# refresh-bio/vclust

Measured on AMD Instinct MI355X. Metric: genome pairs/sec through prefilter+align (ani.tsv), higher is better.
Workload: dtype u64

## Files before the change

### include/vclust_gpu.h

```cpp
#ifndef VCLUST_GPU_H
#define VCLUST_GPU_H

#include <stdint.h>

#ifdef __cplusplus
extern "C" {
#endif

enum {
    VG_OK = 0, VG_EINVAL = -1, VG_EIO = -2, VG_ENODEV = -3, VG_EHIP = -4, VG_ENOMEM = -5,
    VG_EOVERFLOW = -6
};

const char* vg_version(void);
const char* vg_last_error(void);
void        vg_free(void* p);
int vg_device_count(void);
int vg_set_device(int device);
void vg_release_device_memory(void);
int vg_alloc_selftest(const int64_t* sizes, int n_sizes, int cycles);
int vg_copy(void* dst, const void* src, int64_t bytes, int to_host);

typedef struct vg_genomes vg_genomes;

// ... 18 lines not shown
typedef struct { uint32_t a, b, shared; } vg_pair_count;

int vg_kmer_shared(vg_genomes* g, int k, double fraction, int shard, int n_shards,
                   uint32_t min_shared, int64_t* set_sizes, vg_pair_count** pairs,
                   int64_t* n_pairs);
int vg_kmer_shared_new(vg_genomes* g, int n_db, int k, double fraction, uint32_t min_shared, int64_t* set_sizes,
                       vg_pair_count** pairs, int64_t* n_pairs);
void vg_set_new_path(int mode);
typedef struct {
    int accepted; int64_t P; int n_passes;
    int levels, total_bits, B1, B2;
    int st_tiles; int64_t n_st; int u_st, g_st;
    int tile32k, narrow, short_rec;
} vg_kmer_geometry_info;
int vg_kmer_geometry(const vg_genomes* g, int k, double fraction, int shard, int n_shards, vg_kmer_geometry_info* info);
int vg_kmer_geometry_at(int64_t padded_positions, int k, vg_kmer_geometry_info* info);
int vg_rowptr_inline_lo(int64_t entries, int64_t n_genomes, uint32_t* inline_lo);
int vg_kmer_set(vg_genomes* g, int idx, int k, double fraction, uint64_t** out, int64_t* n_out);

int vg_write_fltr(const vg_genomes* g, int k, double fraction, int min_kmers, double min_ident,
                  int max_seqs, const int64_t* set_sizes, const vg_pair_count* pairs,
                  int64_t n_pairs, const char* out_path);

int vg_filter_pairs(int k, int min_kmers, double min_ident, const int64_t* set_sizes, int64_t n_genomes,
                    const vg_pair_count* pairs, int64_t n_pairs, vg_pair_count** out, int64_t* n_out);

typedef struct {
    int    k;
    int    min_kmers;
    double min_ident;
// ... 291 lines not shown
```

### vclust_amd/_lib.py

```python
import collections
import ctypes as C
import os
import pathlib

PKG_DIR = pathlib.Path(__file__).resolve().parent
LIB_PATH = PKG_DIR / 'libvclust_gpu.so'


class VclustGpuError(RuntimeError):
    def __init__(self, code, msg):
        super().__init__(f'libvclust_gpu error {code}: {msg}')
        self.code = code


class PairCount(C.Structure):
    _fields_ = [('a', C.c_uint32), ('b', C.c_uint32), ('shared', C.c_uint32)]


class Task(C.Structure):
    _fields_ = [('q', C.c_uint32), ('r', C.c_uint32)]


class PairStat(C.Structure):
    _fields_ = [('n_match', C.c_uint32), ('aln_len', C.c_uint32), ('n_regions', C.c_uint32)]
# ... 179 lines not shown
    'vg_genomes_count': (C.c_int, [C.c_void_p]),
    'vg_genomes_total_len': (C.c_int64, [C.c_void_p]),
    'vg_genomes_lengths': (C.c_int, [C.c_void_p, P(C.c_int64)]),
    'vg_genomes_name': (C.c_char_p, [C.c_void_p, C.c_int]),
    'vg_genomes_codes': (C.c_int, [C.c_void_p, C.c_int, C.c_void_p]),
    'vg_genomes_to_device': (C.c_int, [C.c_void_p]),
    'vg_genomes_subset': (C.c_int, [C.c_void_p, P(C.c_int32), C.c_int, P(C.c_void_p)]),
    'vg_genomes_extend': (C.c_int, [C.c_void_p, C.c_void_p, P(C.c_int32), C.c_int]),
    'vg_genomes_truncate': (C.c_int, [C.c_void_p, C.c_int]),
    'vg_genomes_reserve': (C.c_int, [C.c_void_p, C.c_int64, C.c_int64]),
    'vg_kmer_shared': (C.c_int, [C.c_void_p, C.c_int, C.c_double, C.c_int, C.c_int, C.c_uint32,
                                 P(C.c_int64), P(P(PairCount)), P(C.c_int64)]),
    'vg_kmer_shared_new': (C.c_int, [C.c_void_p, C.c_int, C.c_int, C.c_double, C.c_uint32, P(C.c_int64), P(P(PairCount)), P(C.c_int64)]),
    'vg_kmer_geometry': (C.c_int, [C.c_void_p, C.c_int, C.c_double, C.c_int, C.c_int, P(KmerGeometry)]),
    'vg_kmer_geometry_at': (C.c_int, [C.c_int64, C.c_int, P(KmerGeometry)]),
    'vg_rowptr_inline_lo': (C.c_int, [C.c_int64, C.c_int64, P(C.c_uint32)]),
    'vg_kmer_set': (C.c_int, [C.c_void_p, C.c_int, C.c_int, C.c_double, P(P(C.c_uint64)), P(C.c_int64)]),
    'vg_filter_pairs': (C.c_int, [C.c_int, C.c_int, C.c_double, C.POINTER(C.c_int64), C.c_int64, C.POINTER(PairCount), C.c_int64,
                                  C.POINTER(C.POINTER(PairCount)), C.POINTER(C.c_int64)]),
    'vg_write_fltr': (C.c_int, [C.c_void_p, C.c_int, C.c_double, C.c_int, C.c_double, C.c_int,
                                P(C.c_int64), P(PairCount), C.c_int64, C.c_char_p]),
    'vg_prefilter': (C.c_int, [P(C.c_char_p), C.c_int, C.c_char_p, P(PrefilterParams)]),
    'vg_prefilter_new': (C.c_int, [P(C.c_char_p), C.c_int, P(C.c_char_p), C.c_int, C.c_char_p, P(PrefilterParams)]),
    'vg_set_process_ends_after_call': (None, [C.c_int]),
    'vg_set_lz_fit': (None, [P(LzFit)]),
    'vg_lz_align': (C.c_int, [C.c_void_p, P(Task), C.c_int64, P(LzParams), P(PairStat),
                              P(P(Region)), P(C.c_int64)]),
    'vg_align_order': (C.c_int, [C.c_void_p, P(C.c_int32)]),
    'vg_read_filter': (C.c_int, [C.c_void_p, C.c_char_p, C.c_double, P(P(PairCount)), P(C.c_int64)]),
    'vg_align_tasks': (C.c_int, [C.c_void_p, P(PairCount), C.c_int64, P(P(Task)), P(C.c_int64)]),
# ... 136 lines not shown
```

### vclust_amd/api.py

```python
import ctypes as C
import inspect

import numpy as np

from . import _lib
from ._lib import (ALIGN_FIELDS, ALIGN_OUTFMT, CLUSTER_ALGORITHMS, LINKAGE_ALGORITHMS, UPDATE_ALGORITHMS, ClusterStat, ClusterStats,
                   ClusterUpdateStats, DedupStats, DerepStats, DerepUpdateStats, KernelTime, LinkageStats, MclParams, MclStats, PairCount,
                   PairStat, Region, Task, as_dict, check, lz_params, path, path_array, ptr)
from .stages import (DEFAULT_LZ, align, align_params, cluster, cluster_stats, deduplicate as deduplicate_files, derep_params, dereplicate,
                     prefilter)


def _dtype(ctype):
    d = np.dtype(ctype)
    return np.dtype(d.descr) if d.names else d


PAIR_DTYPE, TASK_DTYPE, STAT_DTYPE, REGION_DTYPE, CLUSTER_STAT_DTYPE = (_dtype(t) for t in (PairCount, Task, PairStat, Region, ClusterStat))
LINKAGE_DTYPE = np.dtype([('node_a', '<i8'), ('node_b', '<i8'), ('similarity', '<f8'), ('size', '<i8'), ('object_a', '<i4'),
                          ('object_b', '<i4')])
AVERAGE_LINKAGE_DTYPE = np.dtype(LINKAGE_DTYPE.descr + [('sum', '<u8'), ('pairs', '<u8')])


def _input(x, ctype):
# ... 152 lines not shown
        pp, npairs = C.POINTER(PairCount)(), C.c_int64()
        sizes, = _filled(len(self), (C.c_int64,), lambda sp: check(self._lib.vg_kmer_shared(
            self._h, k, float(fraction), shard, n_shards, int(min_shared), sp, C.byref(pp), C.byref(npairs))))
        return sizes, _take(pp, npairs.value, PAIR_DTYPE)

    def kmer_shared_new(self, n_db, k=25, fraction=1.0, min_shared=1):
        pp, npairs = C.POINTER(PairCount)(), C.c_int64()
        sizes, = _filled(len(self), (C.c_int64,), lambda sp: check(self._lib.vg_kmer_shared_new(
            self._h, int(n_db), k, float(fraction), int(min_shared), sp, C.byref(pp), C.byref(npairs))))
        return sizes, _take(pp, npairs.value, PAIR_DTYPE)

    def kmer_geometry(self, k=25, fraction=1.0, shard=0, n_shards=1):
        info = _lib.KmerGeometry()
        check(self._lib.vg_kmer_geometry(self._h, int(k), float(fraction), int(shard), int(n_shards), C.byref(info)))
        return as_dict(info)

    def kmer_set(self, idx, k=25, fraction=1.0):
        p = C.POINTER(C.c_uint64)()
        n = C.c_int64()
        check(self._lib.vg_kmer_set(self._h, idx, k, float(fraction), C.byref(p), C.byref(n)))
        return _take(p, n.value, np.dtype('<u8'))

    def filter_pairs(self, set_sizes, pairs, k=25, min_kmers=20, min_ident=0.7):
        out, n = C.POINTER(PairCount)(), C.c_int64()
        check(self._lib.vg_filter_pairs(int(k), int(min_kmers), float(min_ident), *_input(set_sizes, C.c_int64), *_input(pairs, PairCount),
                                        C.byref(out), C.byref(n)))
        return _take(out, n.value, PAIR_DTYPE)

    def write_fltr(self, out_path, set_sizes, pairs, k=25, fraction=1.0, min_kmers=20, min_ident=0.7, max_seqs=0):
        check(self._lib.vg_write_fltr(self._h, k, float(fraction), int(min_kmers), float(min_ident), int(max_seqs),
# ... 273 lines not shown
```

### vclust_amd/csrc/vg_prefilter.hip

```cpp
#include "vg_common.h"
#include <functional>
#include <map>
#include <mutex>
#include <optional>
#include <rocprim/rocprim.hpp>
#include <algorithm>
#include <cmath>
#include <cstring>

namespace {

constexpr uint64_t SENT = ~0ULL;
constexpr uint32_t SCRAMBLE32 = 0x9E3779B1u;
__host__ __device__ __forceinline__ uint64_t scramble_key(uint64_t cano, int k) {
    const uint32_t L = (uint32_t)cano & ((1u << k) - 1u);
    const uint32_t H = (uint32_t)(cano >> k);
    return ((uint64_t)(H ^ ((L * SCRAMBLE32) >> (32 - k))) << k) | L;
}
__host__ __device__ __forceinline__ uint64_t unscramble_key(uint64_t key, int k) { return scramble_key(key, k); }
constexpr uint32_t DUP_BIT = 0x80000000u;
__device__ __forceinline__ uint32_t rowptr_inline(uint32_t partner) { return 0xFFFFFFFFu - partner; }
__device__ __forceinline__ uint32_t rowptr_partner_of_rs(uint32_t rs) { return 0xFFFFFFFEu - rs; }

__device__ __forceinline__ uint64_t mix64(uint64_t x) {
// ... 1263 lines not shown
                        const uint64_t r = short_rec_pack(key, short_kr, v[2] - grp_row0);
                        __builtin_memcpy(o_rec + 2 * dst, &r, 8);
                    } else __builtin_memcpy(o_rec + 3 * dst, v, 12);
                }
                lds_sync();
                cursors_advance(cursor, thist, nbins);
                lds_sync();
            }
        }
    }
}

constexpr int NT_TILE = 16384;
constexpr int NT_PER = NT_TILE / PT_THREADS;
constexpr int NT_MAXBINS = 2048;
template <bool SHORT>
__global__ void __launch_bounds__(PT_THREADS)
k_part_scatter2_narrow(const uint32_t* __restrict__ rec, int B1, int B2, int64_t n_units, const uint32_t* __restrict__ Ts, lvl2_tab L,
                       uint32_t* __restrict__ o_rec, int narrow_shift) {
    __shared__ uint2 s_rec[NT_TILE];
    __shared__ uint32_t thist[NT_MAXBINS], tstart[NT_MAXBINS], cursor[NT_MAXBINS];
    __shared__ uint32_t s_wave[16];
    const int nbins = 1 << B2;
    const int lane = threadIdx.x & 63, wv = threadIdx.x >> 6;
    for (int64_t u = blockIdx.x; u < n_units; u += gridDim.x) {
        uint32_t b1, U; int64_t s0, s1;
        lvl2_unit(L, u, &b1, &U, &s0, &s1);
        uint32_t gbase = 0, gb[3] = {0, 0, 0};
        uint32_t grow0 = 0, grow1 = 0, grow2 = 0, grow3 = 0;
        if (SHORT) {
            lvl2_groups(L, b1, U, s1, &gbase, gb);
            if (L.wbase) {
                const int64_t w0 = (int64_t)(gbase >> 6), gw = SR_GROUP_WORDS;
                grow0 = L.wbase[min(w0, L.W)]; grow1 = L.wbase[min(w0 + gw, L.W)]; grow2 = L.wbase[min(w0 + 2 * gw, L.W)]; grow3 = L.wbase[min(w0 + 3 * gw, L.W)];
            }
        }
        lds_sync();
        for (int b = threadIdx.x; b < nbins; b += PT_THREADS) cursor[b] = Ts[((uint64_t)b1 * L.n_u + U) * nbins + b];
        for (int64_t t0 = s0; t0 < s1; t0 += NT_TILE) {
            for (int b = threadIdx.x; b < nbins; b += PT_THREADS) thist[b] = 0;
            lds_sync();
            uint32_t key[NT_PER], pay[NT_PER], br[NT_PER];
            if (SHORT) {
                uint4 rr[NT_PER / 2];
#pragma unroll
                for (int p = 0; p < NT_PER / 2; ++p) {
                    const int64_t i = t0 + 2 * ((int64_t)p * PT_THREADS + threadIdx.x);
                    rr[p] = make_uint4(0u, 0u, 0u, 0u);
                    if (i + 1 < s1) __builtin_memcpy(&rr[p], rec + 2 * i, 16);
                    else if (i < s1) __builtin_memcpy(&rr[p].x, rec + 2 * i, 8);
                }
#pragma unroll
                for (int p = 0; p < NT_PER / 2; ++p) {
// ... 33 lines not shown
                uint32_t cn[BPT], tot = 0;
#pragma unroll
                for (int v = 0; v < BPT; ++v) { const int b = BPT * (int)threadIdx.x + v; cn[v] = b < nbins ? thist[b] : 0u; tot += cn[v]; }
                uint32_t run = block_scan_1024(tot, s_wave, nullptr);
#pragma unroll
                for (int v = 0; v < BPT; ++v) { const int b = BPT * (int)threadIdx.x + v; if (b < nbins) tstart[b] = run; run += cn[v]; }
            }
            lds_sync();
#pragma unroll
            for (int j = 0; j < NT_PER; ++j) if (br[j] != 0xffffffffu) s_rec[tstart[br[j] & 0x7ffu] + (br[j] >> 11)] = make_uint2(key[j], pay[j]);
            lds_sync();
            const int per_wave = (nbins + 15) >> 4;
            for (int bb = wv * per_wave; bb < min(nbins, (wv + 1) * per_wave); bb += 8) {
                const int b = bb + (lane >> 3);
                const bool live = b < min(nbins, (wv + 1) * per_wave);
                const uint32_t st = live ? tstart[b] : 0u, cnt = live ? thist[b] : 0u;
                const uint64_t cur = live ? cursor[b] : 0ull;
                for (uint32_t i = (uint32_t)(lane & 7); __any(i < cnt); i += 8) {
                    if (i < cnt) { const uint2 v = s_rec[st + i]; __builtin_memcpy(o_rec + 2 * (cur + i), &v, 8); }
                }
            }
            lds_sync();
            for (int b = threadIdx.x; b < nbins; b += PT_THREADS) cursor[b] += thist[b];
            lds_sync();
        }
    }
}

constexpr int SC_SLAB = 128;
__global__ void __launch_bounds__(PT_THREADS)
k_scan_columns_a(const uint32_t* __restrict__ T, int64_t n_rows, int n_cols, uint32_t* __restrict__ S) {
    const int64_t r0 = (int64_t)blockIdx.x * SC_SLAB, r1 = min(n_rows, r0 + SC_SLAB);
    for (int c = threadIdx.x; c < n_cols; c += PT_THREADS) {
        uint32_t sum = 0;
        for (int64_t r = r0; r < r1; ++r) sum += T[r * n_cols + c];
        S[(int64_t)blockIdx.x * n_cols + c] = sum;
    }
}
__global__ void __launch_bounds__(PT_THREADS)
// ... 52 lines not shown
        uint32_t acc = run;
        for (int u = 0; u < n_u; ++u) { const uint32_t t = tab[(size_t)u * nb2 + c]; tab[(size_t)u * nb2 + c] = acc; acc += t; }
        run += tot[v];
    }
    if (b1 == nb1 - 1 && threadIdx.x == 0) boff[(size_t)nb1 * nb2] = off1[nb1];
}

constexpr int BK_PER = BK_CAP / BK_THREADS;
constexpr int BK_MAXBIN = 768;
template <bool NARROW, int THREADS, int SUBBITS>
__global__ void __launch_bounds__(THREADS)
k_bucket_runs(const uint32_t* __restrict__ rec, int stride ,
              const uint32_t* __restrict__ boff, int64_t n_buckets, int pbits, const uint32_t* __restrict__ blk2g, int blk_shift,
              uint32_t* __restrict__ gen, uint32_t* __restrict__ rowinfo, compact_map M, int* __restrict__ dup_per_genome,
              const uint32_t* __restrict__ bucket_list ,
              uint32_t* __restrict__ over_list, unsigned int* __restrict__ n_over, uint32_t inline_lo) {
    constexpr int BK_SUB = 1 << SUBBITS, CAP = THREADS * BK_PER;
    const uint32_t inline_rank = inline_lo ? 1u : 0u;
    static_assert(CAP <= 8192 && BK_MAXBIN <= 1024, "slot | rank << 13 of the run members");
    __shared__ uint32_t s_big;
    __shared__ uint64_t sk[CAP];
    __shared__ uint32_t sp[NARROW ? 1 : CAP];
    __shared__ uint32_t sgen[CAP];
    __shared__ uint32_t cnt[BK_SUB + 1], start[BK_SUB + 1];
    __shared__ uint32_t s_wave[THREADS / 64];
    const int lane = threadIdx.x & 63, wv = threadIdx.x >> 6;
    for (int64_t it = blockIdx.x; it < n_buckets; it += gridDim.x) {
        const int64_t bk = bucket_list ? (int64_t)bucket_list[it] : it;
        const uint32_t b0 = boff[bk], b1 = boff[bk + 1];
        const uint32_t n_u = b1 - b0;
        if (n_u <= 1) continue;
        if (n_u > (uint32_t)CAP) { if (threadIdx.x == 0) over_list[atomicAdd(n_over, 1u)] = (uint32_t)bk; continue; }
        const int n = (int)n_u;
        lds_sync();
        for (int b = threadIdx.x; b <= BK_SUB; b += THREADS) cnt[b] = 0;
        if (threadIdx.x == 0) s_big = 0;
        lds_sync();
        uint64_t key[BK_PER]; uint32_t pj[BK_PER]; uint32_t sb[BK_PER], ar[BK_PER];
        if (NARROW) {
            static_assert(BK_PER % 2 == 0, "pairs of records per thread");
#pragma unroll
            for (int p = 0; p < BK_PER / 2; ++p) {
                const int j = 2 * (p * THREADS + (int)threadIdx.x);
                uint4 rr = make_uint4(0u, 0u, 0u, 0u);
                if (j + 1 < n) __builtin_memcpy(&rr, rec + 2 * (uint64_t)(b0 + j), 16);
                else if (j < n) __builtin_memcpy(&rr.x, rec + 2 * (uint64_t)(b0 + j), 8);
#pragma unroll
                for (int h = 0; h < 2; ++h) {
                    const int q = 2 * p + h;
                    const uint32_t a = h ? rr.z : rr.x, pay = h ? rr.w : rr.y;
                    sb[q] = 0; ar[q] = 0; key[q] = 0; pj[q] = 0;
                    if (j + h < n) { pj[q] = pay; key[q] = ((uint64_t)a << 32) | pay; sb[q] = a >> (32 - SUBBITS); }
                }
            }
        } else {
#pragma unroll
            for (int q = 0; q < BK_PER; ++q) {
                const int j = q * THREADS + threadIdx.x;
                sb[q] = 0; ar[q] = 0; key[q] = 0; pj[q] = 0;
                if (j < n) {
                    const uint32_t* r = rec + (uint64_t)(b0 + j) * stride;
                    const uint32_t a = r[0], c = stride == 3 ? r[1] : 0u;
                    pj[q] = r[stride - 1];
                    key[q] = ((uint64_t)a << 32) | c;
                    sb[q] = (uint32_t)((key[q] << pbits) >> (64 - SUBBITS));
                }
            }
        }
        auto rec_of = [&](int q) -> int { return NARROW ? 2 * ((q >> 1) * THREADS + (int)threadIdx.x) + (q & 1) : q * THREADS + (int)threadIdx.x; };
#pragma unroll
        for (int q = 0; q < BK_PER; ++q) if (rec_of(q) < n) ar[q] = atomicAdd(&cnt[sb[q]], 1u);
        lds_sync();
        {
            constexpr int CPT = BK_SUB / THREADS;
            uint32_t c4[CPT], tot = 0;
#pragma unroll
// ... 94 lines not shown
    __syncthreads();
    uint32_t base = *carry, tot = *carry;
#pragma unroll
    for (int i = 0; i < BB_THREADS / 64; ++i) { const uint32_t t = s_w[i]; if (i < wv) base = max(base, t); tot = max(tot, t); }
    const uint32_t r = max(base, x);
    __syncthreads();
    if (threadIdx.x == 0) *carry = tot;
    __syncthreads();
    return r;
}
__global__ void __launch_bounds__(BB_THREADS)
k_bucket_big(const uint32_t* __restrict__ rec, int stride, const uint32_t* __restrict__ boff, const uint32_t* __restrict__ list,
             const uint64_t* __restrict__ soff , int pbits,
             uint64_t* __restrict__ kA, uint32_t* __restrict__ pA, uint64_t* __restrict__ kB, uint32_t* __restrict__ pB,
             const uint32_t* __restrict__ blk2g, int blk_shift, uint32_t* __restrict__ gen, uint32_t* __restrict__ rowinfo,
             compact_map M, int* __restrict__ dup_per_genome, uint32_t inline_lo) {
    __shared__ uint32_t hist[BB_DIGITS][256];
    __shared__ uint32_t gbase[256];
    __shared__ uint32_t wcnt[BB_THREADS / 64][256];
    __shared__ uint32_t s_w[BB_THREADS / 64];
    __shared__ uint32_t s_carry_a, s_carry_b;
    const int lane = threadIdx.x & 63, wv = threadIdx.x >> 6;
    const uint32_t bk = list[blockIdx.x];
    const uint32_t b0 = boff[bk];
    const uint32_t n = boff[bk + 1] - b0;
    uint64_t* k0 = kA + soff[blockIdx.x]; uint32_t* p0 = pA + soff[blockIdx.x];
    uint64_t* k1 = kB + soff[blockIdx.x]; uint32_t* p1 = pB + soff[blockIdx.x];
    for (int i = threadIdx.x; i < BB_DIGITS * 256; i += BB_THREADS) (&hist[0][0])[i] = 0;
    __syncthreads();
    for (uint32_t i = threadIdx.x; i < n; i += BB_THREADS) {
        const uint32_t* r = rec + (uint64_t)(b0 + i) * stride;
        uint64_t key; uint32_t pos;
        if (stride == 2) { key = r[0]; pos = r[1]; }
        else { key = ((((uint64_t)r[0] << 32) | r[1]) << pbits) >> pbits; pos = r[2]; }
        k0[i] = key; p0[i] = pos;
#pragma unroll
        for (int d = 0; d < 4; ++d) atomicAdd(&hist[d][(pos >> (8 * d)) & 255u], 1u);
#pragma unroll
        for (int d = 0; d < 8; ++d) atomicAdd(&hist[4 + d][(uint32_t)(key >> (8 * d)) & 255u], 1u);
    }
    __syncthreads();
    for (int d = 0; d < BB_DIGITS; ++d) {
        bool trivial = false;
        if (threadIdx.x < 256 && hist[d][threadIdx.x] == n) trivial = true;
        if (__syncthreads_or(trivial)) continue;
        if (threadIdx.x < 64) {
// ... 81 lines not shown

struct max_op { __device__ __host__ uint32_t operator()(uint32_t a, uint32_t b) const { return a > b ? a : b; } };

}

static int g_force_subshards = 0;
static const char* pf_switch(const char* name) { const char* e = vg_dev_getenv(name); return e ? e : ""; }
static const struct {
    bool radix = !strcmp(pf_switch("VG_INDEX_PATH"), "radix");
    bool long_rec = !strcmp(pf_switch("VG_LEVEL1_RECORDS"), "long");
    bool old_scatter = !strcmp(pf_switch("VG_DENSE_SCATTER"), "staged");
    bool range_dense = !strcmp(pf_switch("VG_RANGE_SCATTER"), "dense");
    bool staged2 = !strcmp(pf_switch("VG_LEVEL2_SCATTER"), "staged");
    bool scan_each = !strcmp(pf_switch("VG_SUBSHARD_SCAN"), "each");
    bool no_inline = !strcmp(pf_switch("VG_ROWPTR_INLINE"), "0");
    int subshards = atoi(pf_switch("VG_SUBSHARDS"));
    int placement_trials = atoi(pf_switch("VG_PLACEMENT_TRIALS"));
    double workspace_gb = [] { const char* e = getenv("VG_WORKSPACE_GB"); const double v = e ? atof(e) : 0.0; return v > 0.01 ? v : 8.0; }();
} g_sw{};
static uint32_t rowptr_inline_lo(uint64_t entries, int64_t n_genomes) {
    if (g_sw.no_inline || n_genomes < 1 || entries >= (1ULL << 32) || (uint64_t)n_genomes >= (1ULL << 32)) return 0u;
    const uint64_t lo = (1ULL << 32) - (uint64_t)n_genomes;
    return entries < lo ? (uint32_t)lo : 0u;
}
template <class F> static void with_k(bool k25, F f) { if (k25) f(std::integral_constant<int, 25>{}); else f(std::integral_constant<int, 0>{}); }
constexpr double SUB_PASS_KMERS = 3.6e9, SUB_PASS_START = 3.9e9;

static bool range_shards(int64_t P, double fraction, int n_shards) {
    return n_shards > 1 && n_shards <= 256 && !(fraction < 1.0) && P < (1LL << 32);
}
// ... 247 lines not shown
    }
    if (W_total > 0) hipLaunchKernelGGL(k_mask_popc, dim3(grid_for(W_total)), dim3(256), 0, s, (const unsigned long long*)wave_mask, W_total, wave_cnt);
    VG_HIP(hipStreamSynchronize(s));
}

struct kmer_index {
    sorted_index si;
    dbuf<uint32_t> arena;
    dbuf<uint32_t> rowinfo, gen; dbuf<int> d_dups;
    std::vector<int> kept, dups;
    int64_t nv = 0, n_rows_info = 0;
    uint32_t inline_lo = 0;
    bool compact_rows = false, rows_from_map = false;
    const uint32_t* wbase = nullptr;
};
struct bucket_geometry {
    bool range, big_buckets, narrow, tile32k, short_rec;
    int total_bits, B1, B2, levels, bin_lo, nb1g, nb1, nb2, st_tiles, n_slabs; int64_t n_st, nbk;
    lvl2_tab L2;
};
static bool bucket_geometry_for(int k, bool dense, const kmer_args& A, int64_t n_src, bucket_geometry& G) {
    G.range = dense && A.dig_n < (1u << DIG_BITS);
    if (g_sw.radix || n_src < (1 << 16) || n_src >= (1LL << 32)) return false;
    const int64_t n_expect = dense && !G.range ? n_src / std::max<uint32_t>(1u, A.n_shards) : n_src;
    if (!bucket_digits(n_expect, &G.total_bits, &G.B1, &G.B2)) return false;
    G.big_buckets = (n_expect >> G.total_bits) > 1024; G.levels = G.total_bits > 11 ? 2 : 1;
    if (G.range && G.B1 > DIG_BITS) return false;
    G.bin_lo = G.range ? (int)(A.dig_lo >> (DIG_BITS - G.B1)) : 0;
    G.nb1g = 1 << G.B1; G.nb2 = 1 << G.B2;
    G.nb1 = G.range ? (int)(((A.dig_lo + A.dig_n - 1) >> (DIG_BITS - G.B1)) - (uint32_t)G.bin_lo + 1) : G.nb1g;
    G.nbk = G.levels == 1 ? G.nb1 : (int64_t)G.nb1 * G.nb2;
    G.narrow = G.levels == 2 && 2 * k - G.total_bits <= 32;
// ... 2 lines not shown
    const int64_t st_pos = (int64_t)G.st_tiles * PT_TILE;
    G.n_st = (n_src + st_pos - 1) / st_pos; G.n_slabs = (int)((G.n_st + SC_SLAB - 1) / SC_SLAB);
    lvl2_tab& L2 = G.L2; memset(&L2, 0, sizeof L2);
    L2.n_st = G.n_st; L2.nb1 = G.nb1; L2.kr = 2 * k - G.B1;
    L2.u_st = (int)std::max<int64_t>(1, std::min<int64_t>(G.n_st, (65536LL * G.nb1g) / st_pos)); L2.n_u = (int)((G.n_st + L2.u_st - 1) / L2.u_st);
    { int sh = 0; while ((1LL << sh) < st_pos) ++sh; L2.st_shift = sh; }
    G.tile32k = dense && G.st_tiles % 4 == 0 && G.B1 <= 12 && !g_sw.old_scatter;
    G.short_rec = G.levels == 2 && G.tile32k && G.narrow && G.B2 <= 11 && L2.kr + SR_POS_BITS <= 64 && L2.kr - G.B2 >= 1 &&
                  (st_pos & (st_pos - 1)) == 0 && st_pos <= (1LL << SR_POS_BITS) && !g_sw.long_rec;
    if (G.short_rec) {
        const int64_t g_st = (1LL << SR_POS_BITS) / st_pos;
        if (L2.u_st <= g_st) L2.g_st = (g_st % L2.u_st == 0) ? 0 : -1;
        else L2.g_st = (L2.u_st % g_st == 0 && L2.u_st / g_st <= 4) ? (int)g_st : -1;
        if (L2.g_st < 0) { G.short_rec = false; L2.g_st = 0; }
    }
    return true;
}
struct bucket_run {
    vg_genomes* g; int k; bool dense; const pass_inputs& in; kmer_index& ix; int* d_kept; hipStream_t s;
    bucket_geometry G; part_src S; compact_map cmap;
    bool k25 = false; uint32_t n1 = 0; size_t n_cap = 0;
    const uint32_t* f_rec = nullptr; int f_stride = 3;
    dbuf<uint32_t> T1s, slab, d_off1, a_rec, b_rec;
    struct ev_guard { hipEvent_t e = nullptr; hipStream_t st; ~ev_guard() { if (e) { (void)hipStreamWaitEvent(st, e, 0); (void)hipEventDestroy(e); } } } rows_zero;
    dbuf<uint32_t> boff;
};
struct level1_tmp { std::optional<vg_prof_scope> ps; dbuf<uint32_t> wave_cnt; dbuf<char> scan_tmp; };
static void clear_rows_aside(bucket_run& R) {
    if (!(R.G.levels == 2 && R.dense && !R.G.range)) return;
    dbuf<uint32_t>& rowinfo = R.ix.rowinfo; const int64_t n_rows_info = R.ix.n_rows_info; hipEvent_t& ev_rows_zero = R.rows_zero.e;
    static const size_t tot = [] { size_t fr0 = 0, t0 = 0; return hipMemGetInfo(&fr0, &t0) == hipSuccess ? t0 : (size_t)0; }();
    if (tot && (size_t)n_rows_info * 4 * 8 <= tot / 2) try {
        { vg_dev_try_scope opportunistic; rowinfo.alloc((size_t)n_rows_info); }
        hipStream_t side = vg_side_stream();
        hipEvent_t ev_s = nullptr;
        VG_HIP(hipEventCreateWithFlags(&ev_s, hipEventDisableTiming));
        VG_HIP(hipEventRecord(ev_s, R.s));
// ... 63 lines not shown
    const size_t n_cap = R.n_cap, rows_cap = G.range ? n_cap : (size_t)R.ix.n_rows_info;
    R.a_rec.alloc(G.levels == 2 ? std::max((G.short_rec ? 2 : 3) * n_cap + 8, rows_cap + n_cap + 16) : 3 * n_cap + 8);
    const int grid_s = (int)std::min<int64_t>(G.n_st, 256);
    const uint32_t* T1s = R.T1s.p; uint32_t* a_rec = R.a_rec.p;
    const int tsh = G.short_rec ? G.L2.kr : 0;
    const bool tile64k = G.st_tiles % 8 == 0 && (uint64_t)A.dig_n * 6 <= (1u << DIG_BITS);
    if (G.tile32k && G.range && G.nb1 <= RG_MAXBINS && !g_sw.range_dense) {
        const bool kc = R.k == 25 && !A.use_frac;
        if (tile64k) with_k(kc, [&](auto K) { hipLaunchKernelGGL((k_part_scatter_range<K(), 65536>), dim3(grid_s), dim3(PT_THREADS), 0, s, S, G.B1, G.nb1, G.st_tiles / 8, G.n_st, T1s, a_rec, tsh); });
        else with_k(kc, [&](auto K) { hipLaunchKernelGGL((k_part_scatter_range<K(), 32768>), dim3(grid_s), dim3(PT_THREADS), 0, s, S, G.B1, G.nb1, G.st_tiles / 4, G.n_st, T1s, a_rec, tsh); });
    }
    else if (G.tile32k) with_k(R.k25 && !G.range, [&](auto K) { hipLaunchKernelGGL(k_part_scatter_dense<K()>, dim3(grid_s), dim3(PT_THREADS), 0, s, S, G.B1, G.nb1, G.st_tiles / 4, G.n_st, T1s, a_rec, tsh); });
    else if (R.dense) hipLaunchKernelGGL((k_part_scatter<SRC_DENSE, 1>), dim3(grid_s), dim3(PT_THREADS), 0, s, S, G.B1, 0, G.st_tiles, G.n_st, T1s, lvl2_tab{}, a_rec, -1, G.nb1);
    else hipLaunchKernelGGL((k_part_scatter<SRC_ARRAYS, 1>), dim3(grid_s), dim3(PT_THREADS), 0, s, S, G.B1, 0, G.st_tiles, G.n_st, T1s, lvl2_tab{}, a_rec, -1, G.nb1);
}
static void level2(bucket_run& R) {
    const bucket_geometry& G = R.G; const lvl2_tab& L2 = G.L2; hipStream_t s = R.s; kmer_index& ix = R.ix;
    const int64_t n_units = (int64_t)G.nb1 * L2.n_u;
    const size_t t2n = (size_t)G.nb1 * (size_t)G.nb2 * (size_t)L2.n_u;
    dbuf<uint32_t> T2s(t2n);
    const uint32_t* a_rec = R.a_rec.p;
    {
        vg_prof_scope ps("kmer_partition2", (double)R.n1 * (4.0 + (G.short_rec ? 8.0 : 12.0) + (G.narrow ? 8.0 : 12.0)));
        const int grid_c2 = (int)std::min<int64_t>(n_units, 512);
        hipLaunchKernelGGL(G.short_rec ? k_part_count2<true> : k_part_count2<false>, dim3(grid_c2), dim3(PT_THREADS), 0, s, a_rec, G.B1, G.B2, n_units, L2, T2s.p);
        hipLaunchKernelGGL(k_scan_units, dim3(G.nb1), dim3(PT_THREADS), 0, s, T2s.p, L2.n_u, G.nb2, (const uint32_t*)R.d_off1.p, G.nb1, R.boff.p);
        R.b_rec.alloc((G.narrow ? 2 : 3) * R.n_cap + 8);
        const int grid_s2 = (int)std::min<int64_t>(n_units, 256);
        if (G.short_rec || (G.narrow && G.B2 <= 11 && !g_sw.staged2))
            hipLaunchKernelGGL(G.short_rec ? k_part_scatter2_narrow<true> : k_part_scatter2_narrow<false>, dim3(grid_s2), dim3(PT_THREADS), 0, s, a_rec, G.B1, G.B2, n_units,
                               (const uint32_t*)T2s.p, L2, R.b_rec.p, G.total_bits);
        else {
            part_src S2; memset(&S2, 0, sizeof S2);
            S2.rec = a_rec; S2.n = (int64_t)R.n1; S2.k2 = 2 * R.k;
            hipLaunchKernelGGL((k_part_scatter<SRC_PLANES, 2>), dim3(grid_s2), dim3(PT_THREADS), 0, s, S2, G.B1, G.B2, 0, n_units,
                               (const uint32_t*)T2s.p, L2, R.b_rec.p, G.narrow ? G.total_bits : -1, 0);
        }
    }
    VG_HIP(hipStreamSynchronize(s));
    vg_host_mark("buckets: level 2 done");
    vg_deferred_start();
    R.f_rec = R.b_rec.p; R.f_stride = G.narrow ? 2 : 3;
    ix.arena = std::move(R.a_rec);
    if (!R.rows_zero.e) ix.rowinfo.view(ix.arena.p, (size_t)ix.n_rows_info);
    ix.gen.view(ix.arena.p + (((size_t)ix.n_rows_info + 3) & ~(size_t)3), (size_t)R.n1 + 4);
}
static void bucket_kernels(bucket_run& R) {
    const bucket_geometry& G = R.G; hipStream_t s = R.s; vg_genomes* g = R.g; kmer_index& ix = R.ix;
    const uint32_t n1 = R.n1; const int64_t nbk = G.nbk;
    if (ix.gen.n < (size_t)n1 + 4) ix.gen.alloc((size_t)n1 + 4);
    if (ix.rowinfo.n < (size_t)ix.n_rows_info) ix.rowinfo.alloc((size_t)ix.n_rows_info);
    ix.inline_lo = rowptr_inline_lo((uint64_t)ix.gen.n, g->n);
    dbuf<unsigned int> d_nover(2); d_nover.zero(s);
    dbuf<uint32_t> over1((size_t)nbk), over2;
    if (R.rows_zero.e) VG_HIP(hipStreamWaitEvent(s, R.rows_zero.e, 0));
    else VG_HIP(hipMemsetAsync(ix.rowinfo.p, 0, (size_t)ix.n_rows_info * sizeof(uint32_t), s));
    const int pb = G.narrow ? 0 : G.total_bits;
    const uint32_t* boff = R.boff.p; const uint32_t* blk2g = g->d_blk2g.p;
    unsigned int n_over[2] = {0, 0};
    auto runs = [&](auto kern, int threads, int grid, int64_t count, const uint32_t* list, uint32_t* over, unsigned int* nover) {
        hipLaunchKernelGGL(kern, dim3(grid), dim3(threads), 0, s, R.f_rec, R.f_stride, boff, count, pb, blk2g, g->align_shift, ix.gen.p, ix.rowinfo.p, R.cmap, ix.d_dups.p, list, over, nover, ix.inline_lo);
    };
    const auto wide = G.narrow ? k_bucket_runs<true, 1024, 11> : k_bucket_runs<false, 1024, 11>;
    {
        vg_prof_scope ps("bucket_sort_runs", (double)n1 * ((G.narrow ? 8 : 12) + 4 + 8));
        const int grid_b = (int)std::min<int64_t>(nbk, 256 * 16);
        if (G.big_buckets) runs(wide, 1024, grid_b, nbk, nullptr, over1.p, d_nover.p);
        else runs(G.narrow ? k_bucket_runs<true, BK_THREADS, 9> : k_bucket_runs<false, BK_THREADS, 9>, BK_THREADS, grid_b, nbk, nullptr, over1.p, d_nover.p);
        d_nover.download(n_over, 2, s);
        VG_HIP(hipStreamSynchronize(s));
    }
    const uint32_t* big_list = over1.p; unsigned int n_big = n_over[0];
    if (n_big > 0 && !G.big_buckets) {
        over2.alloc((size_t)n_big);
        vg_prof_scope ps("bucket_sort_runs_wide", 0);
        runs(wide, 1024, (int)std::min<int64_t>(n_big, 256 * 16), n_big, over1.p, over2.p, d_nover.p + 1);
// ... 2 lines not shown
        big_list = over2.p; n_big = n_over[1];
    }
    if (n_big == 0) return;
    dbuf<uint32_t> d_sz(n_big); std::vector<uint32_t> sz(n_big);
    hipLaunchKernelGGL(k_bucket_sizes, dim3(grid_for(n_big)), dim3(256), 0, s, boff, big_list, (int64_t)n_big, d_sz.p);
    d_sz.download(sz.data(), n_big, s);
    VG_HIP(hipStreamSynchronize(s));
    std::vector<uint64_t> so(n_big); uint64_t tot = 0;
    for (unsigned int i = 0; i < n_big; ++i) { so[i] = tot; tot += ((uint64_t)sz[i] + 3) & ~3ULL; }
    dbuf<uint64_t> d_so(n_big);
    d_so.upload(so.data(), n_big, s);
    dbuf<uint64_t> kA((size_t)tot + 4), kB((size_t)tot + 4); dbuf<uint32_t> pA((size_t)tot + 4), pB((size_t)tot + 4);
    {
        vg_prof_scope ps("bucket_big", (double)tot * 12.0 * 2.0);
        hipLaunchKernelGGL(k_bucket_big, dim3(n_big), dim3(BB_THREADS), 0, s, R.f_rec, R.f_stride, boff, big_list,
                           (const uint64_t*)d_so.p, pb, kA.p, pA.p, kB.p, pB.p, blk2g, g->align_shift, ix.gen.p, ix.rowinfo.p, R.cmap, ix.d_dups.p, ix.inline_lo);
    }
    VG_HIP(hipStreamSynchronize(s));
}
enum class level1 { declined, empty, records };
template <class F> static level1 open_bucket_run(bucket_run& R, const kmer_args& A, F beside) {
    const bool dense = R.dense; const int k = R.k; kmer_index& ix = R.ix;
    R.rows_zero.st = R.s;
    const int64_t n_src = dense ? R.g->padded_total() : ix.nv;
    if (!bucket_geometry_for(k, dense, A, n_src, R.G)) return level1::declined;
    const bucket_geometry& G = R.G;
    R.S.A = A; R.S.keys = dense ? nullptr : ix.si.keys.p; R.S.pos = nullptr; R.S.n = n_src; R.S.k2 = 2 * k; R.S.bin_lo = G.bin_lo;
    R.cmap = dense ? compact_map{ nullptr, nullptr } : compact_map{ ix.si.goff.p, ix.si.cblk.p };
    R.k25 = dense && k == 25 && !A.use_frac && A.n_shards == 1;
    R.T1s.alloc((size_t)G.nb1 * (size_t)G.n_st + 1); R.slab.alloc((size_t)G.n_slabs * G.nb1); R.d_off1.alloc((size_t)G.nb1 + 1);
    R.G.L2.T1s = R.T1s.p; R.G.L2.off1 = R.d_off1.p;
// ... 566 lines not shown
    int rc = vg_genomes_to_device(g); if (rc) throw vg_error(rc, vg_last_error());
    *n_pairs = 0;
    if (g->n == 0) return;
    const shard_plan plan = plan_shards(g, fraction, n_shards, false);
    if (mode_out) *mode_out = plan.range ? 1 : 2;
    unsigned long long n = 0; std::vector<vg_pair_count> none;
    run_passes(shard_call{ g, k, fraction, shard, n_shards, min_shared, 0, xs }, plan, set_sizes, none, &pairs, &n);
    if (!plan.one_pass && !pairs.p) pairs.alloc(1);
    *n_pairs = (int64_t)n;
}

static_assert(sizeof(vg_pair_count) == 12, "pair record layout");
extern "C" void vg_set_subshards(int n) { g_force_subshards = n; }
extern "C" void vg_set_range_scan(int mode) { g_range_scan_mode = mode == 1 ? 1 : 0; }

static void report_geometry(int k, bool dense, const kmer_args& A, int64_t P, vg_kmer_geometry_info* info) {
    bucket_geometry G;
    info->accepted = dense ? (bucket_geometry_for(k, true, A, P, G) ? 1 : 0) : -1;
    if (info->accepted != 1) return;
    info->levels = G.levels; info->total_bits = G.total_bits; info->B1 = G.B1; info->B2 = G.B2;
    info->st_tiles = G.st_tiles; info->n_st = G.n_st; info->u_st = G.L2.u_st; info->g_st = G.L2.g_st;
    info->tile32k = G.tile32k; info->narrow = G.narrow; info->short_rec = G.short_rec;
}
extern "C" int vg_kmer_geometry(const vg_genomes* g, int k, double fraction, int shard, int n_shards, vg_kmer_geometry_info* info) {
    VG_API_BEGIN
    if (!g || !info) throw vg_error(VG_EINVAL, "vg_kmer_geometry: null argument");
    check_kmer_args(k, fraction, shard, n_shards);
    memset(info, 0, sizeof *info);
    const int64_t P = g->padded_total();
    info->P = P; info->n_passes = 1;
    if (g->n == 0) return VG_OK;
    const shard_plan plan = plan_shards(g, fraction, n_shards, true);
    info->n_passes = plan.sub;
    const int sh = shard * plan.sub, ns = n_shards * plan.sub;
    const bool masked = subshards_share_scan(g, fraction, n_shards, plan.sub);
    const bool dense = pass_source_dense(P, fraction, ns, masked);
    report_geometry(k, dense, shard_kmer_args(P, g->align_shift, k, 1.0, sh, ns), P, info);
    VG_API_END
}
extern "C" int vg_kmer_geometry_at(int64_t padded_positions, int k, vg_kmer_geometry_info* info) {
    VG_API_BEGIN
    if (!info) throw vg_error(VG_EINVAL, "vg_kmer_geometry_at: null argument");
    check_kmer_args(k);
    if (padded_positions < 0) throw vg_error(VG_EINVAL, "vg_kmer_geometry_at: negative number of positions");
    memset(info, 0, sizeof *info);
    info->P = padded_positions; info->n_passes = 1;
    report_geometry(k, true, shard_kmer_args(padded_positions, 0, k, 1.0, 0, 1), padded_positions, info);
    VG_API_END
}
extern "C" int vg_rowptr_inline_lo(int64_t entries, int64_t n_genomes, uint32_t* inline_lo) {
    VG_API_BEGIN
    if (!inline_lo) throw vg_error(VG_EINVAL, "vg_rowptr_inline_lo: null argument");
// ... 44 lines not shown
```

Before: 2.711 million.

## Scatter level-2 buckets in one pass into fixed-capacity slots, falling back on overflow

Adds a one-pass level-2 partition. Each level-1 bucket's records go straight into fixed-capacity per-bucket slots sized from the expected occupancy (mean plus 7 standard deviations). This removes the separate count kernel, per-unit scan and second read of the records. The downstream bucket kernels index records by bucket times capacity, and offsets come from a scan of the per-bucket counts. It costs up to 1.5x more scatter buffer memory. On overflow it reruns the counted path, so a run that overflows pays for both passes.

```diff
diff --git a/include/vclust_gpu.h b/include/vclust_gpu.h
--- a/include/vclust_gpu.h
+++ b/include/vclust_gpu.h
@@ -56,6 +56,7 @@
     int tile32k, narrow, short_rec;
 } vg_kmer_geometry_info;
 int vg_kmer_geometry(const vg_genomes* g, int k, double fraction, int shard, int n_shards, vg_kmer_geometry_info* info);
+int vg_kmer_level2_slots(const vg_genomes* g, int k, double fraction, int shard, int n_shards, int* slots);
 int vg_kmer_geometry_at(int64_t padded_positions, int k, vg_kmer_geometry_info* info);
 int vg_rowptr_inline_lo(int64_t entries, int64_t n_genomes, uint32_t* inline_lo);
 int vg_kmer_set(vg_genomes* g, int idx, int k, double fraction, uint64_t** out, int64_t* n_out);
diff --git a/vclust_amd/_lib.py b/vclust_amd/_lib.py
--- a/vclust_amd/_lib.py
+++ b/vclust_amd/_lib.py
@@ -217,6 +217,7 @@
     'vg_kmer_shared_new': (C.c_int, [C.c_void_p, C.c_int, C.c_int, C.c_double, C.c_uint32, P(C.c_int64), P(P(PairCount)), P(C.c_int64)]),
     'vg_kmer_geometry': (C.c_int, [C.c_void_p, C.c_int, C.c_double, C.c_int, C.c_int, P(KmerGeometry)]),
     'vg_kmer_geometry_at': (C.c_int, [C.c_int64, C.c_int, P(KmerGeometry)]),
+    'vg_kmer_level2_slots': (C.c_int, [C.c_void_p, C.c_int, C.c_double, C.c_int, C.c_int, P(C.c_int)]),
     'vg_rowptr_inline_lo': (C.c_int, [C.c_int64, C.c_int64, P(C.c_uint32)]),
     'vg_kmer_set': (C.c_int, [C.c_void_p, C.c_int, C.c_int, C.c_double, P(P(C.c_uint64)), P(C.c_int64)]),
     'vg_filter_pairs': (C.c_int, [C.c_int, C.c_int, C.c_double, C.POINTER(C.c_int64), C.c_int64, C.POINTER(PairCount), C.c_int64,
diff --git a/vclust_amd/api.py b/vclust_amd/api.py
--- a/vclust_amd/api.py
+++ b/vclust_amd/api.py
@@ -190,6 +190,11 @@
         info = _lib.KmerGeometry()
         check(self._lib.vg_kmer_geometry(self._h, int(k), float(fraction), int(shard), int(n_shards), C.byref(info)))
         return as_dict(info)
+
+    def kmer_level2_slots(self, k=25, fraction=1.0, shard=0, n_shards=1):
+        slots = C.c_int(0)
+        check(self._lib.vg_kmer_level2_slots(self._h, int(k), float(fraction), int(shard), int(n_shards), C.byref(slots)))
+        return int(slots.value)
 
     def kmer_set(self, idx, k=25, fraction=1.0):
         p = C.POINTER(C.c_uint64)()
diff --git a/vclust_amd/csrc/vg_prefilter.hip b/vclust_amd/csrc/vg_prefilter.hip
--- a/vclust_amd/csrc/vg_prefilter.hip
+++ b/vclust_amd/csrc/vg_prefilter.hip
@@ -1301,18 +1301,28 @@
 constexpr int NT_TILE = 16384;
 constexpr int NT_PER = NT_TILE / PT_THREADS;
 constexpr int NT_MAXBINS = 2048;
-template <bool SHORT>
+template <bool SHORT, bool ONEPASS>
 __global__ void __launch_bounds__(PT_THREADS)
 k_part_scatter2_narrow(const uint32_t* __restrict__ rec, int B1, int B2, int64_t n_units, const uint32_t* __restrict__ Ts, lvl2_tab L,
-                       uint32_t* __restrict__ o_rec, int narrow_shift) {
+                       uint32_t* __restrict__ o_rec, int narrow_shift, uint32_t cap, uint32_t* __restrict__ cnt2, uint32_t* __restrict__ stat) {
     __shared__ uint2 s_rec[NT_TILE];
     __shared__ uint32_t thist[NT_MAXBINS], tstart[NT_MAXBINS], cursor[NT_MAXBINS];
     __shared__ uint32_t s_wave[16];
+    __shared__ uint32_t s_stop;
     const int nbins = 1 << B2;
     const int lane = threadIdx.x & 63, wv = threadIdx.x >> 6;
-    for (int64_t u = blockIdx.x; u < n_units; u += gridDim.x) {
+    const int64_t bucket_step = ((int64_t)gridDim.x - 1) * L.n_u;
+    for (int64_t u = ONEPASS ? (int64_t)blockIdx.x * L.n_u : (int64_t)blockIdx.x; u < n_units; u += ONEPASS ? 1 + ((u + 1) % L.n_u ? 0 : bucket_step) : (int64_t)gridDim.x) {
         uint32_t b1, U; int64_t s0, s1;
         lvl2_unit(L, u, &b1, &U, &s0, &s1);
+        const uint64_t obase = ONEPASS ? (uint64_t)b1 * (uint64_t)nbins * cap : 0ull;
+        if (ONEPASS && U == 0) {
+            lds_sync();
+            if (threadIdx.x == 0) s_stop = __hip_atomic_load(stat, __ATOMIC_RELAXED, __HIP_MEMORY_SCOPE_AGENT);
+            for (int b = threadIdx.x; b < nbins; b += PT_THREADS) cursor[b] = (uint32_t)b * cap;
+            lds_sync();
+            if (s_stop) break;
+        }
         uint32_t gbase = 0, gb[3] = {0, 0, 0};
         uint32_t grow0 = 0, grow1 = 0, grow2 = 0, grow3 = 0;
         if (SHORT) {
@@ -1323,7 +1333,7 @@
             }
         }
         lds_sync();
-        for (int b = threadIdx.x; b < nbins; b += PT_THREADS) cursor[b] = Ts[((uint64_t)b1 * L.n_u + U) * nbins + b];
+        if (!ONEPASS) for (int b = threadIdx.x; b < nbins; b += PT_THREADS) cursor[b] = Ts[((uint64_t)b1 * L.n_u + U) * nbins + b];
         for (int64_t t0 = s0; t0 < s1; t0 += NT_TILE) {
             for (int b = threadIdx.x; b < nbins; b += PT_THREADS) thist[b] = 0;
             lds_sync();
@@ -1387,15 +1397,27 @@
             for (int bb = wv * per_wave; bb < min(nbins, (wv + 1) * per_wave); bb += 8) {
                 const int b = bb + (lane >> 3);
                 const bool live = b < min(nbins, (wv + 1) * per_wave);
-                const uint32_t st = live ? tstart[b] : 0u, cnt = live ? thist[b] : 0u;
-                const uint64_t cur = live ? cursor[b] : 0ull;
+                const uint32_t st = live ? tstart[b] : 0u; uint32_t cnt = live ? thist[b] : 0u;
+                const uint64_t cur = obase + (live ? cursor[b] : 0u);
+                if (ONEPASS && live) {
+                    const uint32_t room = (uint32_t)(b + 1) * cap - cursor[b];
+                    if (cnt > room) { cnt = room; if ((lane & 7) == 0) stat[0] = 1u; }
+                }
                 for (uint32_t i = (uint32_t)(lane & 7); __any(i < cnt); i += 8) {
                     if (i < cnt) { const uint2 v = s_rec[st + i]; __builtin_memcpy(o_rec + 2 * (cur + i), &v, 8); }
                 }
             }
             lds_sync();
-            for (int b = threadIdx.x; b < nbins; b += PT_THREADS) cursor[b] += thist[b];
+            if (ONEPASS) for (int b = threadIdx.x; b < nbins; b += PT_THREADS) cursor[b] = min(cursor[b] + thist[b], (uint32_t)(b + 1) * cap);
+            else for (int b = threadIdx.x; b < nbins; b += PT_THREADS) cursor[b] += thist[b];
             lds_sync();
+        }
+        if (ONEPASS && U + 1 == (uint32_t)L.n_u) {
+            uint32_t mx = 0;
+            for (int b = threadIdx.x; b < nbins; b += PT_THREADS) { const uint32_t c = cursor[b] - (uint32_t)b * cap; cnt2[(uint64_t)b1 * nbins + b] = c; mx = max(mx, c); }
+#pragma unroll
+            for (int o = 32; o > 0; o >>= 1) mx = max(mx, (uint32_t)__shfl_xor((int)mx, o));
+            if (lane == 0 && mx > 0) atomicMax(&stat[1], mx);
         }
     }
 }
@@ -1478,7 +1500,8 @@
               const uint32_t* __restrict__ boff, int64_t n_buckets, int pbits, const uint32_t* __restrict__ blk2g, int blk_shift,
               uint32_t* __restrict__ gen, uint32_t* __restrict__ rowinfo, compact_map M, int* __restrict__ dup_per_genome,
               const uint32_t* __restrict__ bucket_list ,
-              uint32_t* __restrict__ over_list, unsigned int* __restrict__ n_over, uint32_t inline_lo) {
+              uint32_t* __restrict__ over_list, unsigned int* __restrict__ n_over, uint32_t inline_lo,
+              uint32_t cap ) {
     constexpr int BK_SUB = 1 << SUBBITS, CAP = THREADS * BK_PER;
     const uint32_t inline_rank = inline_lo ? 1u : 0u;
     static_assert(CAP <= 8192 && BK_MAXBIN <= 1024, "slot | rank << 13 of the run members");
@@ -1496,6 +1519,7 @@
         if (n_u <= 1) continue;
         if (n_u > (uint32_t)CAP) { if (threadIdx.x == 0) over_list[atomicAdd(n_over, 1u)] = (uint32_t)bk; continue; }
         const int n = (int)n_u;
+        const uint64_t r0 = cap ? (uint64_t)bk * cap : (uint64_t)b0;
         lds_sync();
         for (int b = threadIdx.x; b <= BK_SUB; b += THREADS) cnt[b] = 0;
         if (threadIdx.x == 0) s_big = 0;
@@ -1507,8 +1531,8 @@
             for (int p = 0; p < BK_PER / 2; ++p) {
                 const int j = 2 * (p * THREADS + (int)threadIdx.x);
                 uint4 rr = make_uint4(0u, 0u, 0u, 0u);
-                if (j + 1 < n) __builtin_memcpy(&rr, rec + 2 * (uint64_t)(b0 + j), 16);
-                else if (j < n) __builtin_memcpy(&rr.x, rec + 2 * (uint64_t)(b0 + j), 8);
+                if (j + 1 < n) __builtin_memcpy(&rr, rec + 2 * (r0 + j), 16);
+                else if (j < n) __builtin_memcpy(&rr.x, rec + 2 * (r0 + j), 8);
 #pragma unroll
                 for (int h = 0; h < 2; ++h) {
                     const int q = 2 * p + h;
@@ -1523,7 +1547,7 @@
                 const int j = q * THREADS + threadIdx.x;
                 sb[q] = 0; ar[q] = 0; key[q] = 0; pj[q] = 0;
                 if (j < n) {
-                    const uint32_t* r = rec + (uint64_t)(b0 + j) * stride;
+                    const uint32_t* r = rec + (r0 + j) * stride;
                     const uint32_t a = r[0], c = stride == 3 ? r[1] : 0u;
                     pj[q] = r[stride - 1];
                     key[q] = ((uint64_t)a << 32) | c;
@@ -1648,7 +1672,7 @@
              const uint64_t* __restrict__ soff , int pbits,
              uint64_t* __restrict__ kA, uint32_t* __restrict__ pA, uint64_t* __restrict__ kB, uint32_t* __restrict__ pB,
              const uint32_t* __restrict__ blk2g, int blk_shift, uint32_t* __restrict__ gen, uint32_t* __restrict__ rowinfo,
-             compact_map M, int* __restrict__ dup_per_genome, uint32_t inline_lo) {
+             compact_map M, int* __restrict__ dup_per_genome, uint32_t inline_lo, uint32_t cap ) {
     __shared__ uint32_t hist[BB_DIGITS][256];
     __shared__ uint32_t gbase[256];
     __shared__ uint32_t wcnt[BB_THREADS / 64][256];
@@ -1658,12 +1682,13 @@
     const uint32_t bk = list[blockIdx.x];
     const uint32_t b0 = boff[bk];
     const uint32_t n = boff[bk + 1] - b0;
+    const uint64_t r0 = cap ? (uint64_t)bk * cap : (uint64_t)b0;
     uint64_t* k0 = kA + soff[blockIdx.x]; uint32_t* p0 = pA + soff[blockIdx.x];
     uint64_t* k1 = kB + soff[blockIdx.x]; uint32_t* p1 = pB + soff[blockIdx.x];
     for (int i = threadIdx.x; i < BB_DIGITS * 256; i += BB_THREADS) (&hist[0][0])[i] = 0;
     __syncthreads();
     for (uint32_t i = threadIdx.x; i < n; i += BB_THREADS) {
-        const uint32_t* r = rec + (uint64_t)(b0 + i) * stride;
+        const uint32_t* r = rec + (r0 + i) * stride;
         uint64_t key; uint32_t pos;
         if (stride == 2) { key = r[0]; pos = r[1]; }
         else { key = ((((uint64_t)r[0] << 32) | r[1]) << pbits) >> pbits; pos = r[2]; }
@@ -1775,6 +1800,8 @@
     bool staged2 = !strcmp(pf_switch("VG_LEVEL2_SCATTER"), "staged");
     bool scan_each = !strcmp(pf_switch("VG_SUBSHARD_SCAN"), "each");
     bool no_inline = !strcmp(pf_switch("VG_ROWPTR_INLINE"), "0");
+    bool l2_counted = !strcmp(pf_switch("VG_LEVEL2"), "counted");
+    int l2_cap = !strncmp(pf_switch("VG_LEVEL2"), "onepass:", 8) ? atoi(pf_switch("VG_LEVEL2") + 8) : 0;
     int subshards = atoi(pf_switch("VG_SUBSHARDS"));
     int placement_trials = atoi(pf_switch("VG_PLACEMENT_TRIALS"));
     double workspace_gb = [] { const char* e = getenv("VG_WORKSPACE_GB"); const double v = e ? atof(e) : 0.0; return v > 0.01 ? v : 8.0; }();
@@ -2052,8 +2079,11 @@
     bool compact_rows = false, rows_from_map = false;
     const uint32_t* wbase = nullptr;
 };
+struct bucket_geometry;
+static uint32_t level2_capacity(const bucket_geometry& G, bool dense, const kmer_args& A, int64_t n_src);
 struct bucket_geometry {
     bool range, big_buckets, narrow, tile32k, short_rec;
+    uint32_t cap2;
     int total_bits, B1, B2, levels, bin_lo, nb1g, nb1, nb2, st_tiles, n_slabs; int64_t n_st, nbk;
     lvl2_tab L2;
 };
@@ -2086,13 +2116,22 @@
         else L2.g_st = (L2.u_st % g_st == 0 && L2.u_st / g_st <= 4) ? (int)g_st : -1;
         if (L2.g_st < 0) { G.short_rec = false; L2.g_st = 0; }
     }
+    G.cap2 = level2_capacity(G, dense, A, n_src);
     return true;
+}
+static uint32_t level2_capacity(const bucket_geometry& G, bool dense, const kmer_args& A, int64_t n_src) {
+    const bool narrow_scatter = G.short_rec || (G.narrow && G.B2 <= 11 && !g_sw.staged2);
+    if (!dense || G.range || A.n_shards != 1 || G.levels != 2 || G.nb1 < 256 || !narrow_scatter || g_sw.l2_counted) return 0u;
+    const double m = (double)n_src / (double)G.nbk;
+    const uint64_t cap = g_sw.l2_cap > 0 ? (uint64_t)g_sw.l2_cap : ((uint64_t)std::ceil(m + 7.0 * std::sqrt(m)) + 7) & ~7ULL;
+    const bool fits = (uint64_t)G.nbk * cap <= (uint64_t)n_src + (uint64_t)n_src / 2 && (uint64_t)G.nb2 * cap < (1ULL << 31);
+    return fits ? (uint32_t)cap : 0u;
 }
 struct bucket_run {
     vg_genomes* g; int k; bool dense; const pass_inputs& in; kmer_index& ix; int* d_kept; hipStream_t s;
     bucket_geometry G; part_src S; compact_map cmap;
     bool k25 = false; uint32_t n1 = 0; size_t n_cap = 0;
-    const uint32_t* f_rec = nullptr; int f_stride = 3;
+    const uint32_t* f_rec = nullptr; int f_stride = 3; uint32_t f_cap = 0;
     dbuf<uint32_t> T1s, slab, d_off1, a_rec, b_rec;
     struct ev_guard { hipEvent_t e = nullptr; hipStream_t st; ~ev_guard() { if (e) { (void)hipStreamWaitEvent(st, e, 0); (void)hipEventDestroy(e); } } } rows_zero;
     dbuf<uint32_t> boff;
@@ -2186,8 +2225,8 @@
     else if (R.dense) hipLaunchKernelGGL((k_part_scatter<SRC_DENSE, 1>), dim3(grid_s), dim3(PT_THREADS), 0, s, S, G.B1, 0, G.st_tiles, G.n_st, T1s, lvl2_tab{}, a_rec, -1, G.nb1);
     else hipLaunchKernelGGL((k_part_scatter<SRC_ARRAYS, 1>), dim3(grid_s), dim3(PT_THREADS), 0, s, S, G.B1, 0, G.st_tiles, G.n_st, T1s, lvl2_tab{}, a_rec, -1, G.nb1);
 }
-static void level2(bucket_run& R) {
-    const bucket_geometry& G = R.G; const lvl2_tab& L2 = G.L2; hipStream_t s = R.s; kmer_index& ix = R.ix;
+static void level2_counted(bucket_run& R) {
+    const bucket_geometry& G = R.G; const lvl2_tab& L2 = G.L2; hipStream_t s = R.s;
     const int64_t n_units = (int64_t)G.nb1 * L2.n_u;
     const size_t t2n = (size_t)G.nb1 * (size_t)G.nb2 * (size_t)L2.n_u;
     dbuf<uint32_t> T2s(t2n);
@@ -2197,11 +2236,11 @@
         const int grid_c2 = (int)std::min<int64_t>(n_units, 512);
         hipLaunchKernelGGL(G.short_rec ? k_part_count2<true> : k_part_count2<false>, dim3(grid_c2), dim3(PT_THREADS), 0, s, a_rec, G.B1, G.B2, n_units, L2, T2s.p);
         hipLaunchKernelGGL(k_scan_units, dim3(G.nb1), dim3(PT_THREADS), 0, s, T2s.p, L2.n_u, G.nb2, (const uint32_t*)R.d_off1.p, G.nb1, R.boff.p);
-        R.b_rec.alloc((G.narrow ? 2 : 3) * R.n_cap + 8);
+        if (!R.b_rec.p) R.b_rec.alloc((G.narrow ? 2 : 3) * R.n_cap + 8);
         const int grid_s2 = (int)std::min<int64_t>(n_units, 256);
         if (G.short_rec || (G.narrow && G.B2 <= 11 && !g_sw.staged2))
-            hipLaunchKernelGGL(G.short_rec ? k_part_scatter2_narrow<true> : k_part_scatter2_narrow<false>, dim3(grid_s2), dim3(PT_THREADS), 0, s, a_rec, G.B1, G.B2, n_units,
-                               (const uint32_t*)T2s.p, L2, R.b_rec.p, G.total_bits);
+            hipLaunchKernelGGL((G.short_rec ? k_part_scatter2_narrow<true, false> : k_part_scatter2_narrow<false, false>), dim3(grid_s2), dim3(PT_THREADS), 0, s, a_rec, G.B1, G.B2, n_units,
+                               (const uint32_t*)T2s.p, L2, R.b_rec.p, G.total_bits, 0u, nullptr, nullptr);
         else {
             part_src S2; memset(&S2, 0, sizeof S2);
             S2.rec = a_rec; S2.n = (int64_t)R.n1; S2.k2 = 2 * R.k;
@@ -2210,9 +2249,35 @@
         }
     }
     VG_HIP(hipStreamSynchronize(s));
+}
+static bool level2_one_pass(bucket_run& R) {
+    const bucket_geometry& G = R.G; const lvl2_tab& L2 = G.L2; hipStream_t s = R.s;
+    const int64_t n_units = (int64_t)G.nb1 * L2.n_u;
+    R.b_rec.alloc(2 * std::max((size_t)G.nbk * G.cap2, R.n_cap) + 8);
+    dbuf<uint32_t> stat(2); stat.zero(s);
+    uint32_t h_stat[2] = {0, 0};
+    {
+        vg_prof_scope ps("kmer_partition2", (double)R.n1 * ((G.short_rec ? 8.0 : 12.0) + 8.0));
+        hipLaunchKernelGGL((G.short_rec ? k_part_scatter2_narrow<true, true> : k_part_scatter2_narrow<false, true>), dim3((unsigned)std::min(G.nb1, 256)), dim3(PT_THREADS), 0, s,
+                           (const uint32_t*)R.a_rec.p, G.B1, G.B2, n_units, nullptr, L2, R.b_rec.p, G.total_bits, G.cap2, R.boff.p, stat.p);
+        VG_HIP(hipMemsetAsync(R.boff.p + G.nbk, 0, sizeof(uint32_t), s));
+        with_temp_storage([&](void* tmp, size_t& tb) { return rocprim::exclusive_scan(tmp, tb, R.boff.p, R.boff.p, 0u, (size_t)G.nbk + 1, rocprim::plus<uint32_t>(), s); });
+    }
+    stat.download(h_stat, 2, s);
+    VG_HIP(hipStreamSynchronize(s));
+    char mark[96];
+    snprintf(mark, sizeof mark, h_stat[0] ? "level2: one pass overflowed, counted (%u slots)" : "level2: one pass (largest bucket %u of %u slots)", h_stat[0] ? G.cap2 : h_stat[1], G.cap2);
+    vg_host_mark(mark);
+    return h_stat[0] == 0;
+}
+static void level2(bucket_run& R) {
+    const bucket_geometry& G = R.G; kmer_index& ix = R.ix;
+    uint32_t cap = G.cap2;
+    if (cap && !level2_one_pass(R)) cap = 0;
+    if (!cap) level2_counted(R);
     vg_host_mark("buckets: level 2 done");
     vg_deferred_start();
-    R.f_rec = R.b_rec.p; R.f_stride = G.narrow ? 2 : 3;
+    R.f_rec = R.b_rec.p; R.f_stride = G.narrow ? 2 : 3; R.f_cap = cap;
     ix.arena = std::move(R.a_rec);
     if (!R.rows_zero.e) ix.rowinfo.view(ix.arena.p, (size_t)ix.n_rows_info);
     ix.gen.view(ix.arena.p + (((size_t)ix.n_rows_info + 3) & ~(size_t)3), (size_t)R.n1 + 4);
@@ -2231,7 +2296,7 @@
     const uint32_t* boff = R.boff.p; const uint32_t* blk2g = g->d_blk2g.p;
     unsigned int n_over[2] = {0, 0};
     auto runs = [&](auto kern, int threads, int grid, int64_t count, const uint32_t* list, uint32_t* over, unsigned int* nover) {
-        hipLaunchKernelGGL(kern, dim3(grid), dim3(threads), 0, s, R.f_rec, R.f_stride, boff, count, pb, blk2g, g->align_shift, ix.gen.p, ix.rowinfo.p, R.cmap, ix.d_dups.p, list, over, nover, ix.inline_lo);
+        hipLaunchKernelGGL(kern, dim3(grid), dim3(threads), 0, s, R.f_rec, R.f_stride, boff, count, pb, blk2g, g->align_shift, ix.gen.p, ix.rowinfo.p, R.cmap, ix.d_dups.p, list, over, nover, ix.inline_lo, R.f_cap);
     };
     const auto wide = G.narrow ? k_bucket_runs<true, 1024, 11> : k_bucket_runs<false, 1024, 11>;
     {
@@ -2264,7 +2329,7 @@
     {
         vg_prof_scope ps("bucket_big", (double)tot * 12.0 * 2.0);
         hipLaunchKernelGGL(k_bucket_big, dim3(n_big), dim3(BB_THREADS), 0, s, R.f_rec, R.f_stride, boff, big_list,
-                           (const uint64_t*)d_so.p, pb, kA.p, pA.p, kB.p, pB.p, blk2g, g->align_shift, ix.gen.p, ix.rowinfo.p, R.cmap, ix.d_dups.p, ix.inline_lo);
+                           (const uint64_t*)d_so.p, pb, kA.p, pA.p, kB.p, pB.p, blk2g, g->align_shift, ix.gen.p, ix.rowinfo.p, R.cmap, ix.d_dups.p, ix.inline_lo, R.f_cap);
     }
     VG_HIP(hipStreamSynchronize(s));
 }
@@ -2861,28 +2926,42 @@
 extern "C" void vg_set_subshards(int n) { g_force_subshards = n; }
 extern "C" void vg_set_range_scan(int mode) { g_range_scan_mode = mode == 1 ? 1 : 0; }
 
-static void report_geometry(int k, bool dense, const kmer_args& A, int64_t P, vg_kmer_geometry_info* info) {
+static void report_geometry(int k, bool dense, const kmer_args& A, int64_t P, vg_kmer_geometry_info* info, int* level2_slots = nullptr) {
     bucket_geometry G;
+    if (level2_slots) *level2_slots = 0;
     info->accepted = dense ? (bucket_geometry_for(k, true, A, P, G) ? 1 : 0) : -1;
     if (info->accepted != 1) return;
     info->levels = G.levels; info->total_bits = G.total_bits; info->B1 = G.B1; info->B2 = G.B2;
     info->st_tiles = G.st_tiles; info->n_st = G.n_st; info->u_st = G.L2.u_st; info->g_st = G.L2.g_st;
+    if (level2_slots) *level2_slots = (int)G.cap2;
     info->tile32k = G.tile32k; info->narrow = G.narrow; info->short_rec = G.short_rec;
 }
-extern "C" int vg_kmer_geometry(const vg_genomes* g, int k, double fraction, int shard, int n_shards, vg_kmer_geometry_info* info) {
-    VG_API_BEGIN
-    if (!g || !info) throw vg_error(VG_EINVAL, "vg_kmer_geometry: null argument");
-    check_kmer_args(k, fraction, shard, n_shards);
+static void first_pass_geometry(const vg_genomes* g, int k, double fraction, int shard, int n_shards, vg_kmer_geometry_info* info, int* level2_slots) {
     memset(info, 0, sizeof *info);
+    if (level2_slots) *level2_slots = 0;
     const int64_t P = g->padded_total();
     info->P = P; info->n_passes = 1;
-    if (g->n == 0) return VG_OK;
+    if (g->n == 0) return;
     const shard_plan plan = plan_shards(g, fraction, n_shards, true);
     info->n_passes = plan.sub;
     const int sh = shard * plan.sub, ns = n_shards * plan.sub;
     const bool masked = subshards_share_scan(g, fraction, n_shards, plan.sub);
     const bool dense = pass_source_dense(P, fraction, ns, masked);
-    report_geometry(k, dense, shard_kmer_args(P, g->align_shift, k, 1.0, sh, ns), P, info);
+    report_geometry(k, dense, shard_kmer_args(P, g->align_shift, k, 1.0, sh, ns), P, info, level2_slots);
+}
+extern "C" int vg_kmer_geometry(const vg_genomes* g, int k, double fraction, int shard, int n_shards, vg_kmer_geometry_info* info) {
+    VG_API_BEGIN
+    if (!g || !info) throw vg_error(VG_EINVAL, "vg_kmer_geometry: null argument");
+    check_kmer_args(k, fraction, shard, n_shards);
+    first_pass_geometry(g, k, fraction, shard, n_shards, info, nullptr);
+    VG_API_END
+}
+extern "C" int vg_kmer_level2_slots(const vg_genomes* g, int k, double fraction, int shard, int n_shards, int* slots) {
+    VG_API_BEGIN
+    if (!g || !slots) throw vg_error(VG_EINVAL, "vg_kmer_level2_slots: null argument");
+    check_kmer_args(k, fraction, shard, n_shards);
+    vg_kmer_geometry_info info;
+    first_pass_geometry(g, k, fraction, shard, n_shards, &info, slots);
     VG_API_END
 }
 extern "C" int vg_kmer_geometry_at(int64_t padded_positions, int k, vg_kmer_geometry_info* info) {
```

Result: faster. 2.939 million, median of 6 (+8.4%).
